# ViTAE-Transformer/LeMeViT

Hardware: AMD Instinct MI355X
Metric: images/sec LeMeViT-Base 224^2 bf16 fwd+bwd (higher is better)
Workload: dtype bf16; 1 GPU; lemevit_base 224x224 bf16-autocast train step (fwd+bwd+AdamW), batch 128/GPU, drop_path 0.1, random-init weights; global_batch=128, parallelism=dp1, launch=eager, weight-gradient GEMMs on a side stream

## Files before the change

### lemevit_amd/csrc/attn_mfma.hip

```cpp
#include <stdlib.h>
#include <atomic>
#include "common.h"
#include "attn_internal.h"

#ifndef LMV_XCD_REMAP
#define LMV_XCD_REMAP 1
#endif

namespace {

constexpr int D = 32;
typedef __attribute__((address_space(3))) bf16x4_t* lds4_t;

__device__ __forceinline__ int swz(int r, int c16) { return r * 64 + ((c16 ^ (((r >> 2) & 1) << 1)) << 4); }

template <int NTHREADS>
__device__ __forceinline__ void stage_rows2(unsigned char* sa, const bf16_t* ba, int64_t rsa, unsigned char* sb, const bf16_t* bb, int64_t rsb,
                                            int r0, int nrows, int L, int tid) {
  const int total = nrows * 4, last = max(L - 1, 0);
  for (int c0 = 0; c0 < total; c0 += NTHREADS * 4) {
    uint4 va[4], vb[4];
#pragma unroll
    for (int j = 0; j < 4; ++j) {
      const int c = min(c0 + j * NTHREADS + tid, total - 1), cc = c & 3;
      const int rr = min(r0 + (c >> 2), last);
      va[j] = *reinterpret_cast<const uint4*>(ba + (int64_t)rr * rsa + cc * 8);
      vb[j] = *reinterpret_cast<const uint4*>(bb + (int64_t)rr * rsb + cc * 8);
    }
#pragma unroll
    for (int j = 0; j < 4; ++j) {
      const int c = c0 + j * NTHREADS + tid, r = c >> 2, cc = c & 3;
      if (c >= total) continue;
      const bool ok = r0 + r < L;
      *reinterpret_cast<uint4*>(sa + swz(r, cc)) = ok ? va[j] : make_uint4(0, 0, 0, 0);
      *reinterpret_cast<uint4*>(sb + swz(r, cc)) = ok ? vb[j] : make_uint4(0, 0, 0, 0);
    }
  }
}

__device__ __forceinline__ bf16x8_t frag_n(const unsigned char* s, int row0, int lane) {
  return *reinterpret_cast<const bf16x8_t*>(s + swz(row0 + (lane & 15), lane >> 4));
}
__device__ __forceinline__ bf16x8_t frag_t(const unsigned char* s, int rowA, int rowB, int d0, int lane) {
  const int g = lane >> 4, i = lane & 15, rr = i >> 2, q = i & 3;
  const int ra = rowA + g * 4 + rr, rb = rowB + g * 4 + rr, c16 = q, off = (d0 >> 4) * 8;
  bf16x4_t lo = __builtin_amdgcn_ds_read_tr16_b64_v4bf16((lds4_t)(s + swz(ra, c16) + off));
  bf16x4_t hi = __builtin_amdgcn_ds_read_tr16_b64_v4bf16((lds4_t)(s + swz(rb, c16) + off));
  return __builtin_shufflevector(lo, hi, 0, 1, 2, 3, 4, 5, 6, 7);
}

__device__ __forceinline__ bf16x8_t pack8(const f32x4_t& a, const f32x4_t& b) {
  bf16x8_t r;
  r[0] = (__bf16)a[0]; r[1] = (__bf16)a[1]; r[2] = (__bf16)a[2]; r[3] = (__bf16)a[3];
  r[4] = (__bf16)b[0]; r[5] = (__bf16)b[1]; r[6] = (__bf16)b[2]; r[7] = (__bf16)b[3];
  return r;
}
__device__ __forceinline__ bf16x8_t load_frag_global(const bf16_t* base, int64_t rs, int row, int L, int lane) {
  uint4 v = make_uint4(0, 0, 0, 0);
  if (row < L) v = *reinterpret_cast<const uint4*>(base + (int64_t)row * rs + (lane >> 4) * 8);
  return __builtin_bit_cast(bf16x8_t, v);
}
__device__ __forceinline__ float group_max4(float v) { return lmv_xmax4(v); }
__device__ __forceinline__ float group_sum4(float v) { return lmv_xsum4(v); }
__device__ __forceinline__ void store4(bf16_t* p, const f32x4_t& v) { *reinterpret_cast<uint2*>(p) = make_uint2(pack_bf2(v[0], v[1]), pack_bf2(v[2], v[3])); }
__device__ __forceinline__ void store8(bf16_t* row, int g, const f32x4_t& x0, const f32x4_t& x1) {
  *reinterpret_cast<uint4*>(row + g * 8) = make_uint4(pack_bf2(x0[0], x0[1]), pack_bf2(x0[2], x0[3]), pack_bf2(x1[0], x1[1]), pack_bf2(x1[2], x1[3]));
}

#define MFMA(a, b, c) __builtin_amdgcn_mfma_f32_16x16x32_bf16(a, b, c, 0, 0, 0)

__device__ __forceinline__ int xcd_contiguous(int id, int n) {
  if (n & 7) return id;
  return (id & 7) * (n >> 3) + (id >> 3);
}

typedef __attribute__((ext_vector_type(8))) _Float16 f16x8_t;
typedef __attribute__((ext_vector_type(2))) _Float16 f16x2_t;

__device__ __forceinline__ unsigned bf2_to_h2(unsigned w) {
  const float lo = fminf(fmaxf(__uint_as_float(w << 16), -65504.f), 65504.f), hi = fminf(fmaxf(__uint_as_float(w & 0xffff0000u), -65504.f), 65504.f);
  return __builtin_bit_cast(unsigned, __builtin_amdgcn_cvt_pkrtz(lo, hi));
}
__device__ __forceinline__ f16x8_t pack8h(const f32x4_t& a, const f32x4_t& b) {
  typedef __attribute__((ext_vector_type(4))) unsigned u32x4_t;
  const u32x4_t w = {__builtin_bit_cast(unsigned, __builtin_amdgcn_cvt_pkrtz(a[0], a[1])), __builtin_bit_cast(unsigned, __builtin_amdgcn_cvt_pkrtz(a[2], a[3])),
                     __builtin_bit_cast(unsigned, __builtin_amdgcn_cvt_pkrtz(b[0], b[1])), __builtin_bit_cast(unsigned, __builtin_amdgcn_cvt_pkrtz(b[2], b[3]))};
  return __builtin_bit_cast(f16x8_t, w);
}

template <int NKT, int LK = 0, bool PV16 = false>
__device__ __forceinline__ void mfma_fwd_body(const AttnArgs& a, int qt_per_block, const int bx, const int h, const int b) {
  __shared__ __attribute__((aligned(16))) unsigned char sK[NKT * 16 * 64], sV[NKT * 16 * 64];
  const int tid = threadIdx.x, lane = tid & 63, wave = tid >> 6;
  const int Lk = LK ? LK : a.Lk;
  const bf16_t* qb = reinterpret_cast<const bf16_t*>(a.q) + b * a.q_bs + h * D;
  const bf16_t* kb = reinterpret_cast<const bf16_t*>(a.k) + b * a.k_bs + h * D;
  const bf16_t* vb = reinterpret_cast<const bf16_t*>(a.v) + b * a.v_bs + h * D;
  bf16_t* ob = reinterpret_cast<bf16_t*>(a.o) + b * a.o_bs + h * D;
  stage_rows2<256>(sK, kb, a.k_rs, sV, vb, a.v_rs, 0, NKT * 16, Lk, tid);
  __syncthreads();
  if constexpr (PV16) {
    for (int c = tid; c < NKT * 16 * 4; c += 256) {
      uint4 v = *reinterpret_cast<const uint4*>(sV + c * 16);
      v.x = bf2_to_h2(v.x); v.y = bf2_to_h2(v.y); v.z = bf2_to_h2(v.z); v.w = bf2_to_h2(v.w);
      *reinterpret_cast<uint4*>(sV + c * 16) = v;
    }
    __syncthreads();
  }
  const int nqt = (a.Lq + 15) >> 4;
  const int qt_end = min(nqt, (bx + 1) * qt_per_block);
  const int g = lane >> 4;
  const float sc2 = a.scale * 1.4426950408889634f;
  bf16x8_t qf_next = load_frag_global(qb, a.q_rs, (bx * qt_per_block + wave) * 16 + (lane & 15), a.Lq, lane);
  for (int qt = bx * qt_per_block + wave; qt < qt_end; qt += 4) {
    const int q = qt * 16 + (lane & 15);
    const bf16x8_t qf = qf_next;
    if (qt + 4 < qt_end) qf_next = load_frag_global(qb, a.q_rs, q + 64, a.Lq, lane);
    f32x4_t s[NKT];
    float m = -3e38f;
#pragma unroll
    for (int kt = 0; kt < NKT; ++kt) {
      if (LK && kt * 16 >= LK) { s[kt] = f32x4_t{-3e38f, -3e38f, -3e38f, -3e38f}; continue; }
      s[kt] = MFMA(frag_n(sK, kt * 16, lane), qf, (f32x4_t{0.f, 0.f, 0.f, 0.f}));
      if (kt * 16 + 16 > Lk) {
#pragma unroll
        for (int r = 0; r < 4; ++r)
          if (kt * 16 + g * 4 + r >= Lk) s[kt][r] = -3e38f;
      }
#pragma unroll
      for (int r = 0; r < 4; ++r) m = fmaxf(m, s[kt][r]);
    }
    m = group_max4(m);
    const float mc = m * sc2;
    float l = 0.f;
#pragma unroll
    for (int kt = 0; kt < NKT; ++kt) {
      if (LK && kt * 16 >= LK) { s[kt] = f32x4_t{0.f, 0.f, 0.f, 0.f}; continue; }
#pragma unroll
      for (int r = 0; r < 4; ++r) { const float p = __builtin_amdgcn_exp2f(fmaf(s[kt][r], sc2, -mc)); s[kt][r] = p; l += p; }
    }
    l = group_sum4(l);
    f32x4_t o0 = {0.f, 0.f, 0.f, 0.f}, o1 = {0.f, 0.f, 0.f, 0.f};
#pragma unroll
    for (int kb2 = 0; kb2 < NKT / 2; ++kb2) {
      if (LK && kb2 * 32 >= LK) continue;
      const bf16x8_t vt0 = frag_t(sV, kb2 * 32, kb2 * 32 + 16, 0, lane), vt1 = frag_t(sV, kb2 * 32, kb2 * 32 + 16, 16, lane);
      if constexpr (PV16) {
        const f16x8_t ph = pack8h(s[2 * kb2], s[2 * kb2 + 1]);
        o0 = __builtin_amdgcn_mfma_f32_16x16x32_f16(__builtin_bit_cast(f16x8_t, vt0), ph, o0, 0, 0, 0);
        o1 = __builtin_amdgcn_mfma_f32_16x16x32_f16(__builtin_bit_cast(f16x8_t, vt1), ph, o1, 0, 0, 0);
      } else {
        const bf16x8_t ph = pack8(s[2 * kb2], s[2 * kb2 + 1]);
        f32x4_t r0, r1;
#pragma unroll
        for (int r = 0; r < 4; ++r) { r0[r] = s[2 * kb2][r] - (float)ph[r]; r1[r] = s[2 * kb2 + 1][r] - (float)ph[4 + r]; }
        const bf16x8_t pl = pack8(r0, r1);
        o0 = MFMA(vt0, ph, o0); o0 = MFMA(vt0, pl, o0);
        o1 = MFMA(vt1, ph, o1); o1 = MFMA(vt1, pl, o1);
      }
    }
    if (q < a.Lq) {
      const float inv = 1.f / l;
      o0 *= inv; o1 *= inv;
      store8(ob + (int64_t)q * a.o_rs, g, o0, o1);
      if (a.lse && g == 0) a.lse[((int64_t)b * a.H + h) * a.Lq + q] = m * a.scale + __logf(l);
    }
  }
}

template <int NKT, int LK = 0, bool PV16 = false>
__global__ __launch_bounds__(256) void mfma_fwd_kernel(const AttnArgs a, int qt_per_block) {
  const int nb = gridDim.x, n = nb * a.H * a.B;
  const int L = LMV_XCD_REMAP ? xcd_contiguous((int)blockIdx.x + nb * ((int)blockIdx.y + a.H * (int)blockIdx.z), n) : (int)blockIdx.x + nb * ((int)blockIdx.y + a.H * (int)blockIdx.z);
  mfma_fwd_body<NKT, LK, PV16>(a, qt_per_block, L % nb, (L / nb) % a.H, L / (nb * a.H));
}

template <int NKT1, int LK1, int NKT2, int LK2>
__global__ __launch_bounds__(256) void mfma_fwd_pair_kernel(const AttnArgs a1, const AttnArgs a2, int per1, int per2, int nblk1) {
  const int n1 = nblk1 * a1.H * a1.B;
  int id = (int)blockIdx.x;
  if (id < n1 && LMV_XCD_REMAP) id = xcd_contiguous(id, n1);
  if (id < n1) { const int bx = id % nblk1, t = id / nblk1; mfma_fwd_body<NKT1, LK1, true>(a1, per1, bx, t % a1.H, t / a1.H); }
  else { const int t = id - n1; mfma_fwd_body<NKT2, LK2, true>(a2, per2, 0, t % a2.H, t / a2.H); }
}

template <int NKT>
__global__ __launch_bounds__(256) void mfma_bwd_dq_kernel(const AttnArgs a, float* __restrict__ delta, int qt_per_block) {
  __shared__ __attribute__((aligned(16))) unsigned char sK[NKT * 16 * 64], sV[NKT * 16 * 64];
  const int tid = threadIdx.x, lane = tid & 63, wave = tid >> 6, h = blockIdx.y, b = blockIdx.z;
  const bf16_t* qb = reinterpret_cast<const bf16_t*>(a.q) + b * a.q_bs + h * D;
  const bf16_t* gb = reinterpret_cast<const bf16_t*>(a.d_o) + b * a.o_bs + h * D;
  const bf16_t* ob = reinterpret_cast<const bf16_t*>(a.o) + b * a.o_bs + h * D;
  bf16_t* dqb = reinterpret_cast<bf16_t*>(a.dq) + b * a.q_bs + h * D;
  stage_rows2<256>(sK, reinterpret_cast<const bf16_t*>(a.k) + b * a.k_bs + h * D, a.k_rs, sV, reinterpret_cast<const bf16_t*>(a.v) + b * a.v_bs + h * D, a.v_rs, 0, NKT * 16, a.Lk, tid);
  __syncthreads();
  const int nqt = (a.Lq + 15) >> 4;
  const int qt_end = min(nqt, (int)(blockIdx.x + 1) * qt_per_block);
  const int g = lane >> 4;
  const int64_t bh = ((int64_t)b * a.H + h) * a.Lq;
  for (int qt = blockIdx.x * qt_per_block + wave; qt < qt_end; qt += 4) {
    const int q = qt * 16 + (lane & 15);
    const bool vq = q < a.Lq;
    const bf16x8_t qf = load_frag_global(qb, a.q_rs, q, a.Lq, lane);
    const bf16x8_t gf = load_frag_global(gb, a.o_rs, q, a.Lq, lane);
    const bf16x8_t of = load_frag_global(ob, a.o_rs, q, a.Lq, lane);
    const float lse = vq ? a.lse[bh + q] : 0.f;
    float dl = 0.f;
#pragma unroll
    for (int j = 0; j < 8; ++j) dl += (float)gf[j] * (float)of[j];
    dl = group_sum4(dl);
    if (vq && g == 0) delta[bh + q] = dl;
    f32x4_t dq0 = {0.f, 0.f, 0.f, 0.f}, dq1 = {0.f, 0.f, 0.f, 0.f};
#pragma unroll
    for (int kb2 = 0; kb2 < NKT / 2; ++kb2) {
      f32x4_t ds[2];
#pragma unroll
      for (int t = 0; t < 2; ++t) {
        const int kt = 2 * kb2 + t;
        const f32x4_t s = MFMA(frag_n(sK, kt * 16, lane), qf, (f32x4_t{0.f, 0.f, 0.f, 0.f}));
        const f32x4_t dp = MFMA(frag_n(sV, kt * 16, lane), gf, (f32x4_t{0.f, 0.f, 0.f, 0.f}));
#pragma unroll
        for (int r = 0; r < 4; ++r) {
          const bool ok = vq && (kt * 16 + g * 4 + r < a.Lk);
          const float p = ok ? __expf(s[r] * a.scale - lse) : 0.f;
          ds[t][r] = p * (dp[r] - dl) * a.scale;
        }
      }
      const bf16x8_t dsf = pack8(ds[0], ds[1]);
      dq0 = MFMA(frag_t(sK, kb2 * 32, kb2 * 32 + 16, 0, lane), dsf, dq0);
      dq1 = MFMA(frag_t(sK, kb2 * 32, kb2 * 32 + 16, 16, lane), dsf, dq1);
    }
    if (vq) {
      store8(dqb + (int64_t)q * a.q_rs, g, dq0, dq1);
    }
  }
}
// ... 364 lines not shown
    const float4 d0 = *reinterpret_cast<const float4*>(sDl + r0 + g * 4), d1 = *reinterpret_cast<const float4*>(sDl + r0 + 16 + g * 4);
    const float lse[8] = {l0.x, l0.y, l0.z, l0.w, l1.x, l1.y, l1.z, l1.w};
    const float dl[8] = {d0.x, d0.y, d0.z, d0.w, d1.x, d1.y, d1.z, d1.w};
#pragma unroll
    for (int i = 0; i < TPW; ++i) {
      const int kt = wave + i * 4;
      if (kt >= NKT || kt * 16 >= Lk) continue;
      const bool kvalid = kt * 16 + (lane & 15) < Lk;
      const f32x4_t s0 = MFMA(qn0, kf[i], (f32x4_t{0.f, 0.f, 0.f, 0.f})), s1 = MFMA(qn1, kf[i], (f32x4_t{0.f, 0.f, 0.f, 0.f}));
      const f32x4_t p0 = MFMA(gn0, vf[i], (f32x4_t{0.f, 0.f, 0.f, 0.f})), p1 = MFMA(gn1, vf[i], (f32x4_t{0.f, 0.f, 0.f, 0.f}));
      f32x4_t pr[2], ds[2];
#pragma unroll
      for (int r = 0; r < 4; ++r) {
        const float e0 = kvalid ? __expf(s0[r] * a.scale - lse[r]) : 0.f, e1 = kvalid ? __expf(s1[r] * a.scale - lse[4 + r]) : 0.f;
        pr[0][r] = e0; pr[1][r] = e1;
        ds[0][r] = e0 * (p0[r] - dl[r]) * a.scale; ds[1][r] = e1 * (p1[r] - dl[4 + r]) * a.scale;
      }
      const bf16x8_t pf = pack8(pr[0], pr[1]), dsf = pack8(ds[0], ds[1]);
      dv[i][0] = MFMA(gt0, pf, dv[i][0]); dv[i][1] = MFMA(gt1, pf, dv[i][1]);
      dk[i][0] = MFMA(qt0, dsf, dk[i][0]); dk[i][1] = MFMA(qt1, dsf, dk[i][1]);
      const uint4 w = __builtin_bit_cast(uint4, dsf);
      const int wsl = (g ^ ((lane >> 2) & 3)) * 8;
      *reinterpret_cast<uint2*>(sT(buf, wave, 0, i) + (lane & 15) * 32 + wsl) = make_uint2(w.x, w.y);
      *reinterpret_cast<uint2*>(sT(buf, wave, 1, i) + (lane & 15) * 32 + wsl) = make_uint2(w.z, w.w);
    }
    __syncthreads();
    {
      const int rr = (lane & 15) >> 2, qq = lane & 3;
      f32x4_t dq = {0.f, 0.f, 0.f, 0.f};
#pragma unroll
      for (int pp = 0; pp < NPAIR; ++pp) {
        const int kta = 2 * pp, ktb = 2 * pp + 1;
        if (kta * 16 >= Lk) continue;
        const bool has_b = ktb < NKT && ktb * 16 < Lk;
        const bf16x4_t lo = __builtin_amdgcn_ds_read_tr16_b64_v4bf16((lds4_t)(sT(buf, kta & 3, qt_w, kta >> 2) + (g * 4 + rr) * 32 + (qq ^ g) * 8));
        bf16x4_t hi = {(__bf16)0.f, (__bf16)0.f, (__bf16)0.f, (__bf16)0.f};
        if (has_b) hi = __builtin_amdgcn_ds_read_tr16_b64_v4bf16((lds4_t)(sT(buf, ktb & 3, qt_w, ktb >> 2) + (g * 4 + rr) * 32 + (qq ^ g) * 8));
        const bf16x8_t dst = __builtin_shufflevector(lo, hi, 0, 1, 2, 3, 4, 5, 6, 7);
        dq = MFMA(ktf[pp], dst, dq);
      }
      const int q = r0 + qt_w * 16 + (lane & 15);
      if (q < Lq) store4(dqb + (int64_t)q * a.q_rs + g * 8 + dh * 4, dq);
    }
  }
#pragma unroll
  for (int i = 0; i < TPW; ++i) {
    const int kt = wave + i * 4, key = kt * 16 + (lane & 15);
    if (kt >= NKT || key >= Lk) continue;
    store8(reinterpret_cast<bf16_t*>(a.dk) + b * a.k_bs + (int64_t)key * a.k_rs + h * D, g, dk[i][0], dk[i][1]);
    store8(reinterpret_cast<bf16_t*>(a.dv) + b * a.v_bs + (int64_t)key * a.v_rs + h * D, g, dv[i][0], dv[i][1]);
  }
}

template <int NKT, int LK = 0, int VER = 1>
__global__ __launch_bounds__(256, 2) void mfma_bwd_fused_kernel(const AttnArgs a) {
  const int n = a.H * a.B, id = (int)blockIdx.y + a.H * (int)blockIdx.z;
  const int L = LMV_XCD_REMAP ? xcd_contiguous(id, n) : id;
  if constexpr (VER == 2) mfma_bwd_fused_body2<NKT, LK>(a, L % a.H, L / a.H);
  else mfma_bwd_fused_body<NKT, LK>(a, L % a.H, L / a.H);
}

template <int NKT1, int LK1, int VER = 1>
__global__ __launch_bounds__(256, 2) void mfma_bwd_pair_kernel(const AttnArgs a1, const AttnArgs a2) {
  const int n1 = a1.H * a1.B;
  int id = (int)blockIdx.x;
  if (id < n1 && LMV_XCD_REMAP) id = xcd_contiguous(id, n1);
  if (id < n1) { if constexpr (VER == 2) mfma_bwd_fused_body2<NKT1, LK1>(a1, id % a1.H, id / a1.H); else mfma_bwd_fused_body<NKT1, LK1>(a1, id % a1.H, id / a1.H); }
  else mfma_bwd_dkv_body<2, 1, false, true, 16, 32>(a2, nullptr, nullptr, nullptr, 32, 0, (id - n1) % a2.H, (id - n1) / a2.H);
}

__global__ __launch_bounds__(256) void scatter_bf16_kernel(const float* __restrict__ acc, bf16_t* __restrict__ dst, int64_t bs, int64_t rs, int B, int H,
                                                          int L, int LP) {
  const unsigned idx = blockIdx.x * 256 + threadIdx.x, total = (unsigned)B * H * L * D;
  if (idx >= total) return;
  const unsigned d = idx % D, l = (idx / D) % L, h = (idx / (D * L)) % H, b = idx / (D * L * H);
  dst[b * bs + (int64_t)l * rs + h * D + d] = f2bf(acc[((((int64_t)b * H + h) * LP) + l) * D + d]);
}

__global__ __launch_bounds__(256) void scatter_sum_kernel(const float* __restrict__ acc0, const float* __restrict__ acc1, bf16_t* __restrict__ dst0,
                                                         bf16_t* __restrict__ dst1, int64_t bs0, int64_t rs0, int64_t bs1, int64_t rs1, int B, int H, int L,
                                                         int LP, int nslab) {
  const unsigned idx = blockIdx.x * 256 + threadIdx.x, per = (unsigned)B * H * L * (D / 4);
  if (idx >= 2 * per) return;
  const bool second = idx >= per;
  const unsigned i = second ? idx - per : idx;
  const unsigned d4 = i % (D / 4), l = (i / (D / 4)) % L, h = (i / ((D / 4) * L)) % H, b = i / ((D / 4) * L * H);
  const float* src = (second ? acc1 : acc0) + ((((int64_t)b * H + h) * LP) + l) * D + d4 * 4;
  const int64_t slab = (int64_t)B * H * LP * D;
  f32x4_t s = {0.f, 0.f, 0.f, 0.f};
  for (int k = 0; k < nslab; ++k) s += *reinterpret_cast<const f32x4_t*>(src + k * slab);
  bf16_t* dst = second ? dst1 + b * bs1 + (int64_t)l * rs1 + h * D + d4 * 4 : dst0 + b * bs0 + (int64_t)l * rs0 + h * D + d4 * 4;
  store4(dst, s);
}

constexpr int RKT = 8, RK = RKT * 16;
constexpr int RKT_B = 4, RKB = RKT_B * 16;

__global__ __launch_bounds__(256) void mfma_fwd_split_kernel(const AttnArgs a, float* __restrict__ part, int nsplit) {
  __shared__ __attribute__((aligned(16))) unsigned char sK[4 * RK * 64], sV[4 * RK * 64];
  const int tid = threadIdx.x, lane = tid & 63, wave = tid >> 6, g = lane >> 4;
  const int nbx = gridDim.x, Lid = LMV_XCD_REMAP ? xcd_contiguous((int)blockIdx.x + nbx * ((int)blockIdx.y + a.H * (int)blockIdx.z), nbx * a.H * a.B)
                                                 : (int)blockIdx.x + nbx * ((int)blockIdx.y + a.H * (int)blockIdx.z);
  const int bx = Lid % nbx, h = (Lid / nbx) % a.H, b = Lid / (nbx * a.H);
  const int split = bx * 4 + wave, k0 = split * RK;
  const bf16_t* kb = reinterpret_cast<const bf16_t*>(a.k) + b * a.k_bs + h * D;
  const bf16_t* vb = reinterpret_cast<const bf16_t*>(a.v) + b * a.v_bs + h * D;
  unsigned char* wK = sK + wave * RK * 64;
  unsigned char* wV = sV + wave * RK * 64;
  stage_rows2<64>(wK, kb, a.k_rs, wV, vb, a.v_rs, k0, RK, a.Lk, lane);
  asm volatile("s_waitcnt vmcnt(0) lgkmcnt(0)" ::: "memory");
  __builtin_amdgcn_wave_barrier();
  if (split >= nsplit) return;
  const int q = lane & 15;
  float* pp = part + ((((int64_t)b * a.H + h) * nsplit + split) * 16 + q) * (D + 2);
  if (k0 >= a.Lk) {
    if (g == 0) { pp[0] = -1e30f; pp[1] = 0.f; }
#pragma unroll
    for (int r = 0; r < 4; ++r) { pp[2 + g * 4 + r] = 0.f; pp[18 + g * 4 + r] = 0.f; }
    return;
  }
// ... 642 lines not shown
    else if (a.Lk == 49) hipLaunchKernelGGL((mfma_bwd_fused_kernel<4, 49>), grid, block, 0, st, a);
    else if (nkt == 4) hipLaunchKernelGGL((mfma_bwd_fused_kernel<4>), grid, block, 0, st, a);
    else if (nkt == 8) hipLaunchKernelGGL((mfma_bwd_fused_kernel<8>), grid, block, 0, st, a);
    else hipLaunchKernelGGL((mfma_bwd_fused_kernel<14>), grid, block, 0, st, a);
    LMV_CHECK_LAUNCH("attn_mfma_bwd_fused");
    return LMV_OK;
  }
  if (nkt == 14 && a.Lq > 16) {
    int nk, pr, lds;
    if (int rc = long_geometry(a, &nk, &pr, &lds)) return rc;
    hipLaunchKernelGGL(mfma_bwd_dq_long_kernel, dim3((nqt + pr - 1) / pr, a.H, a.B), dim3(256), lds, st, a, delta, pr, nk);
  } else if (nkt == 2 && fuse_dq) {
  } else {
    dim3 grid((nqt + per - 1) / per, a.H, a.B), block(256);
    switch (nkt) {
      case 2: hipLaunchKernelGGL((mfma_bwd_dq_kernel<2>), grid, block, 0, st, a, delta, per); break;
      case 4: hipLaunchKernelGGL((mfma_bwd_dq_kernel<4>), grid, block, 0, st, a, delta, per); break;
      case 8: hipLaunchKernelGGL((mfma_bwd_dq_kernel<8>), grid, block, 0, st, a, delta, per); break;
      default: hipLaunchKernelGGL((mfma_bwd_dq_kernel<14>), grid, block, 0, st, a, delta, per); break;
    }
  }
  int nsplit, qpb;
  dkv_split(a, &nsplit, &qpb);
  dim3 grid(nsplit, a.H, a.B), block(256);
  const size_t acc_elems = (size_t)nsplit * a.B * a.H * nkt * 16 * D;
  float* acc_k = acc; float* acc_v = acc + acc_elems;
  if (nsplit > 1) {
#define DKV(N, K) hipLaunchKernelGGL((mfma_bwd_dkv_kernel<N, K, true>), grid, block, 0, st, a, delta, acc_k, acc_v, qpb)
    if (nkt == 2 && fuse_dq && a.Lk == 16) hipLaunchKernelGGL((mfma_bwd_dkv_kernel<2, 1, true, true, 16>), grid, block, 0, st, a, delta, acc_k, acc_v, qpb);
    else if (nkt == 2 && fuse_dq) hipLaunchKernelGGL((mfma_bwd_dkv_kernel<2, 1, true, true>), grid, block, 0, st, a, delta, acc_k, acc_v, qpb);
    else
    switch (nkt) { case 2: DKV(2, 1); break; case 4: DKV(4, 2); break; case 8: DKV(8, 4); break; default: DKV(14, 4); break; }
#undef DKV
    const unsigned n = 2u * (unsigned)a.B * a.H * a.Lk * (D / 4);
    hipLaunchKernelGGL(scatter_sum_kernel, dim3((n + 255) / 256), dim3(256), 0, st, (const float*)acc_k, (const float*)acc_v, (bf16_t*)a.dk, (bf16_t*)a.dv,
                       a.k_bs, a.k_rs, a.v_bs, a.v_rs, a.B, a.H, a.Lk, nkt * 16, nsplit);
  } else {
#define DKV(N, K) hipLaunchKernelGGL((mfma_bwd_dkv_kernel<N, K, false>), grid, block, 0, st, a, delta, acc_k, acc_v, qpb)
    if (nkt == 2 && fuse_dq && a.Lk == 16) hipLaunchKernelGGL((mfma_bwd_dkv_kernel<2, 1, false, true, 16>), grid, block, 0, st, a, delta, acc_k, acc_v, qpb);
    else if (nkt == 2 && fuse_dq) hipLaunchKernelGGL((mfma_bwd_dkv_kernel<2, 1, false, true>), grid, block, 0, st, a, delta, acc_k, acc_v, qpb);
    else
    switch (nkt) { case 2: DKV(2, 1); break; case 4: DKV(4, 2); break; case 8: DKV(8, 4); break; default: DKV(14, 4); break; }
#undef DKV
  }
  LMV_CHECK_LAUNCH("attn_mfma_bwd");
  return LMV_OK;
}

int lmv_attn_mfma_fwd_pair(const AttnArgs& a1, const AttnArgs& a2, hipStream_t st) {
  const int on = lmv_config().attn_pair;
  if (!on || a1.B != a2.B || a1.H != a2.H || a2.Lk != 16 || a2.Lq != 16 || a1.Lq != a1.Lk || (a1.Lk != 196 && a1.Lk != 49)) return 0;
  const int per1 = qt_per_block_for(a1), nqt1 = (a1.Lq + 15) / 16, nblk1 = (nqt1 + per1 - 1) / per1;
  dim3 grid((nblk1 + 1) * a1.H * a1.B), block(256);
  if (a1.Lk == 196) hipLaunchKernelGGL((mfma_fwd_pair_kernel<14, 196, 2, 16>), grid, block, 0, st, a1, a2, per1, 1, nblk1);
  else hipLaunchKernelGGL((mfma_fwd_pair_kernel<4, 49, 2, 16>), grid, block, 0, st, a1, a2, per1, 1, nblk1);
  return 1;
}

int lmv_attn_mfma_bwd_pair(const AttnArgs& a1, const AttnArgs& a2, hipStream_t st) {
  const int on = lmv_config().attn_pair;
  if (!on || a1.B != a2.B || a1.H != a2.H || a2.Lk != 16 || a2.Lq != 16 || a1.Lq != a1.Lk || (a1.Lk != 196 && a1.Lk != 49)) return 0;
  dim3 grid(2 * a1.H * a1.B), block(256);
  const bool v2 = lmv_config().attn_fused_bwd == 2;
  if (a1.Lk == 196 && v2) hipLaunchKernelGGL((mfma_bwd_pair_kernel<14, 196, 2>), grid, block, 0, st, a1, a2);
  else if (v2) hipLaunchKernelGGL((mfma_bwd_pair_kernel<4, 49, 2>), grid, block, 0, st, a1, a2);
  else if (a1.Lk == 196) hipLaunchKernelGGL((mfma_bwd_pair_kernel<14, 196>), grid, block, 0, st, a1, a2);
  else hipLaunchKernelGGL((mfma_bwd_pair_kernel<4, 49>), grid, block, 0, st, a1, a2);
  return 1;
}
```

### lemevit_amd/csrc/common.h

```cpp
#pragma once
#include <hip/hip_runtime.h>
#include <stdint.h>
#include <stdio.h>
#include "../../include/lemevit_hip.h"

typedef unsigned short bf16_t;
typedef __attribute__((ext_vector_type(8))) __bf16 bf16x8_t;
typedef __attribute__((ext_vector_type(4))) __bf16 bf16x4_t;
typedef __attribute__((ext_vector_type(4))) float f32x4_t;

#define LMV_WAVE 64

void lmv_set_error(const char* fmt, ...);
#define LMV_FAIL(code, ...)          \
  do {                               \
    lmv_set_error(__VA_ARGS__);      \
    return (code);                   \
  } while (0)
unsigned* lmv_stage_errword(void* stream);
int lmv_stage_capacity(const void* kernel, int threads, size_t lds_bytes);

extern bool g_lmv_timing_on;
void lmv_timing_begin(void* stream, double flops, double bytes, int kind);
void lmv_timing_end(void* stream);
// ... 18 lines not shown
                                                                float* __restrict__ out_a, int na, float* __restrict__ out_b, int mode) {
  const int cx = threadIdx.x & 7, rg = threadIdx.x >> 3, i = (blk * 8 + cx) * 4;
  float4 a = make_float4(0.f, 0.f, 0.f, 0.f);
  if (i < width) {
    const float* p = partial + i;
    int r = rg;
    for (; r + 96 < nrows; r += 128) {
      const float4 v0 = *reinterpret_cast<const float4*>(p + (int64_t)r * width);
      const float4 v1 = *reinterpret_cast<const float4*>(p + (int64_t)(r + 32) * width);
      const float4 v2 = *reinterpret_cast<const float4*>(p + (int64_t)(r + 64) * width);
      const float4 v3 = *reinterpret_cast<const float4*>(p + (int64_t)(r + 96) * width);
      a.x += (v0.x + v1.x) + (v2.x + v3.x); a.y += (v0.y + v1.y) + (v2.y + v3.y);
      a.z += (v0.z + v1.z) + (v2.z + v3.z); a.w += (v0.w + v1.w) + (v2.w + v3.w);
    }
    for (; r < nrows; r += 32) {
      const float4 v = *reinterpret_cast<const float4*>(p + (int64_t)r * width);
      a.x += v.x; a.y += v.y; a.z += v.z; a.w += v.w;
    }
  }
  red[rg * 8 + cx] = a;
  __syncthreads();
  if (rg == 0 && i < width) {
#pragma unroll 8
    for (int k = 1; k < 32; ++k) { const float4 v = red[k * 8 + cx]; a.x += v.x; a.y += v.y; a.z += v.z; a.w += v.w; }
    const float s[4] = {a.x, a.y, a.z, a.w};
#pragma unroll
    for (int e = 0; e < 4; ++e) {
      const int j = i + e;
      if (mode == 0) { if (j < na) out_a[j] += s[e]; else out_b[j - na] += s[e]; }
      else { const int t = j / na, ch = j - t * na; if (t < 9) out_a[ch * 9 + t] += s[e]; else out_b[ch] += s[e]; }
    }
  }
}

struct LmvConfig {
  int gemm_bk;
  int gemm_bk32_tiles;
  int dw_bk;
  int dw_target_blocks;
  int gemm_no_dma;
  int gemm_w8;
  int gemm_cumap;
  int gemm_nst, gemm_nst_dw;
  int gemm_wn;
  int gemm_rs;
  int dwconv_v;
  int ln_exact_fused;
  int res_ln_fused;
  int dx_ln_fused;
  int mlp_split384;
  int mlp_rw96;
  int mlp_tm;
  int attn_pv16, attn_fuse_dq, attn_fused_bwd, attn_pair;
  int ln_bwd_blocks, ln_bwd_minrows;
  int stage_ticket_skew;
};
LmvConfig& lmv_config();

bool lmv_rs_eligible(const lmv_linear_problem* p, int nproblems, int N, int K, int act, bool force);
int lmv_rs_linear(const lmv_linear_problem* p, int nproblems, int N, int K, int act, hipStream_t st);
bool lmv_wn_eligible(const lmv_linear_problem* p, int nproblems, int N, int K, int act, bool force);
bool lmv_mlp_rw96_eligible(const lmv_mlp_problem* p, int nproblems, int C, int hidden);
int lmv_mlp_rw96_fwd(const lmv_mlp_problem* p, int nproblems, const lmv_mlp_weights* w, float eps, hipStream_t st);
int lmv_wn_linear(const lmv_linear_problem* p, int nproblems, int N, int K, int act, hipStream_t st);

static inline bool lmv_aligned16(const void* p) { return (((uintptr_t)p) & 15u) == 0; }

__device__ __forceinline__ float bf2f(bf16_t v) { return __uint_as_float(((unsigned)v) << 16); }
typedef __attribute__((ext_vector_type(2))) __bf16 bf16x2_t;
typedef __attribute__((ext_vector_type(2))) float f32x2_t;
__device__ __forceinline__ unsigned pack_bf2(float lo, float hi) {
  const f32x2_t f = {lo, hi};
  return __builtin_bit_cast(unsigned, __builtin_convertvector(f, bf16x2_t));
}
__device__ __forceinline__ bf16_t f2bf(float f) { return (bf16_t)(pack_bf2(f, 0.f) & 0xffffu); }

template <typename T> struct DT;
template <> struct DT<float> {
  static constexpr int EPC = 4;
  static __device__ __forceinline__ float ld(const float* p) { return *p; }
  static __device__ __forceinline__ void st(float* p, float v) { *p = v; }
};
template <> struct DT<bf16_t> {
  static constexpr int EPC = 8;
  static __device__ __forceinline__ float ld(const bf16_t* p) { return bf2f(*p); }
  static __device__ __forceinline__ void st(bf16_t* p, float v) { *p = f2bf(v); }
};

template <typename T> __device__ __forceinline__ void chunk_to_f(const uint4& c, float* f);
template <> __device__ __forceinline__ void chunk_to_f<float>(const uint4& c, float* f) {
  f[0] = __uint_as_float(c.x); f[1] = __uint_as_float(c.y); f[2] = __uint_as_float(c.z); f[3] = __uint_as_float(c.w);
}
template <> __device__ __forceinline__ void chunk_to_f<bf16_t>(const uint4& c, float* f) {
  f[0] = __uint_as_float(c.x << 16); f[1] = __uint_as_float(c.x & 0xffff0000u);
  f[2] = __uint_as_float(c.y << 16); f[3] = __uint_as_float(c.y & 0xffff0000u);
  f[4] = __uint_as_float(c.z << 16); f[5] = __uint_as_float(c.z & 0xffff0000u);
  f[6] = __uint_as_float(c.w << 16); f[7] = __uint_as_float(c.w & 0xffff0000u);
}
template <typename T> __device__ __forceinline__ uint4 f_to_chunk(const float* f);
template <> __device__ __forceinline__ uint4 f_to_chunk<float>(const float* f) {
  return make_uint4(__float_as_uint(f[0]), __float_as_uint(f[1]), __float_as_uint(f[2]), __float_as_uint(f[3]));
}
template <> __device__ __forceinline__ uint4 f_to_chunk<bf16_t>(const float* f) {
  return make_uint4(pack_bf2(f[0], f[1]), pack_bf2(f[2], f[3]), pack_bf2(f[4], f[5]), pack_bf2(f[6], f[7]));
}

// ... 68 lines not shown
```

### lemevit_amd/csrc/misc.hip

```cpp
#include <stdarg.h>
#include <string.h>
#include <mutex>
#include <vector>
#include "common.h"

static thread_local char g_err[512] = "";

void lmv_set_error(const char* fmt, ...) {
  va_list ap;
  va_start(ap, fmt);
  vsnprintf(g_err, sizeof(g_err), fmt, ap);
  va_end(ap);
}
extern "C" const char* lmv_last_error(void) { return g_err; }

namespace {
struct ErrWord { unsigned* host = nullptr; unsigned* dev = nullptr; };
ErrWord g_errword[64];
std::mutex g_errword_mu;
}
unsigned* lmv_stage_errword(void* stream) {
  int dev = 0;
  (void)hipGetDevice(&dev);
  std::lock_guard<std::mutex> lock(g_errword_mu);
// ... 42 lines not shown
size_t g_timing_n = 0;
}
void lmv_timing_begin(void* stream, double flops, double bytes, int kind) {
  if (g_timing_n >= g_timing.size()) return;
  TimingRec& r = g_timing[g_timing_n];
  r.flops = flops; r.bytes = bytes; r.kind = kind;
  (void)hipEventRecord(r.e0, (hipStream_t)stream);
}
void lmv_timing_end(void* stream) {
  if (g_timing_n >= g_timing.size()) return;
  (void)hipEventRecord(g_timing[g_timing_n++].e1, (hipStream_t)stream);
}
void lmv_timing_set_kind(int kind) {
  if (g_timing_n < g_timing.size()) g_timing[g_timing_n].kind = kind;
}
extern "C" int lmv_debug_launch_timing(int capacity) {
  g_lmv_timing_on = false;
  for (auto& r : g_timing) { (void)hipEventDestroy(r.e0); (void)hipEventDestroy(r.e1); }
  g_timing.clear(); g_timing_n = 0;
  if (capacity <= 0) return LMV_OK;
  g_timing.resize((size_t)capacity);
  for (auto& r : g_timing)
    if (hipEventCreate(&r.e0) != hipSuccess || hipEventCreate(&r.e1) != hipSuccess) LMV_FAIL(LMV_ERR_LAUNCH, "launch timing: cannot create events");
  g_lmv_timing_on = true;
  return LMV_OK;
}
extern "C" int lmv_debug_launch_timing_read(float* ms, double* flops, double* bytes, int* kinds, int capacity) {
  g_lmv_timing_on = false;
  int n = 0;
  for (size_t i = 0; i < g_timing_n && n < capacity; ++i) {
    float t = 0.f;
    if (hipEventElapsedTime(&t, g_timing[i].e0, g_timing[i].e1) != hipSuccess) continue;
    ms[n] = t; flops[n] = g_timing[i].flops; bytes[n] = g_timing[i].bytes; kinds[n] = g_timing[i].kind; ++n;
  }
  return n;
}

extern "C" int lmv_abi_version(void) { return LMV_ABI_VERSION; }

#include <stdlib.h>
#include <string.h>
namespace {
int env_int(const char* name, int dflt) { const char* e = name ? getenv(name) : nullptr; return e && *e ? atoi(e) : dflt; }
struct ConfigKey { const char* key; const char* env; int LmvConfig::*field; int dflt; };
const ConfigKey kConfigKeys[] = {
    {"gemm_bk", nullptr, &LmvConfig::gemm_bk, 0}, {"gemm_bk32_tiles", nullptr, &LmvConfig::gemm_bk32_tiles, 512},
    {"dw_bk", nullptr, &LmvConfig::dw_bk, 32}, {"dw_target_blocks", "LMV_DW_TARGET_BLOCKS", &LmvConfig::dw_target_blocks, 0},
    {"gemm_no_dma", nullptr, &LmvConfig::gemm_no_dma, 0}, {"gemm_w8", "LMV_GEMM_W8", &LmvConfig::gemm_w8, 1},
    {"gemm_cumap", nullptr, &LmvConfig::gemm_cumap, 1}, {"gemm_nst", nullptr, &LmvConfig::gemm_nst, 2},
    {"gemm_nst_dw", nullptr, &LmvConfig::gemm_nst_dw, 3}, {"gemm_rs", "LMV_GEMM_RS", &LmvConfig::gemm_rs, 1}, {"gemm_wn", "LMV_GEMM_WN", &LmvConfig::gemm_wn, 1},
    {"dwconv_v", nullptr, &LmvConfig::dwconv_v, 0},
    {"stage_ticket_skew", "LMV_STAGE_TICKET_SKEW", &LmvConfig::stage_ticket_skew, 0}, {"mlp_tm", nullptr, &LmvConfig::mlp_tm, 0}, {"mlp_rw96", nullptr, &LmvConfig::mlp_rw96, 1}, {"mlp_split384", nullptr, &LmvConfig::mlp_split384, 1}, {"dx_ln_fused", nullptr, &LmvConfig::dx_ln_fused, 1}, {"res_ln_fused", nullptr, &LmvConfig::res_ln_fused, 1}, {"ln_exact_fused", nullptr, &LmvConfig::ln_exact_fused, 1}, {"attn_pv16", nullptr, &LmvConfig::attn_pv16, 1},
    {"attn_fuse_dq", nullptr, &LmvConfig::attn_fuse_dq, 1}, {"attn_fused_bwd", nullptr, &LmvConfig::attn_fused_bwd, 2},
    {"attn_pair", nullptr, &LmvConfig::attn_pair, 1}, {"ln_bwd_blocks", nullptr, &LmvConfig::ln_bwd_blocks, 1024},
    {"ln_bwd_minrows", nullptr, &LmvConfig::ln_bwd_minrows, 2},
};
LmvConfig config_from_env() {
  LmvConfig c{};
  for (const ConfigKey& k : kConfigKeys) c.*(k.field) = env_int(k.env, k.dflt);
  if (c.ln_bwd_blocks <= 0 || c.ln_bwd_blocks > 2048) c.ln_bwd_blocks = 512;
  if (c.ln_bwd_minrows <= 0) c.ln_bwd_minrows = 2;
  return c;
}
LmvConfig g_config = config_from_env();
}
LmvConfig& lmv_config() { return g_config; }
extern "C" int lmv_config_set(const char* key, int value) {
  if (!key) LMV_FAIL(LMV_ERR_SHAPE, "config_set: null key");
  for (const ConfigKey& k : kConfigKeys)
    if (!strcmp(k.key, key)) { g_config.*(k.field) = value; return LMV_OK; }
  LMV_FAIL(LMV_ERR_SHAPE, "config_set: unknown key '%s'", key);
}
extern "C" int lmv_config_get(const char* key, int* value) {
  if (!key || !value) LMV_FAIL(LMV_ERR_SHAPE, "config_get: null argument");
  for (const ConfigKey& k : kConfigKeys)
    if (!strcmp(k.key, key)) { *value = g_config.*(k.field); return LMV_OK; }
  LMV_FAIL(LMV_ERR_SHAPE, "config_get: unknown key '%s'", key);
}

namespace {

constexpr int TPB = 256;
inline int grid_for(int64_t work_items) {
  int64_t b = (work_items + TPB - 1) / TPB;
  if (b > 2048) b = 2048;
  if (b < 1) b = 1;
  return (int)b;
}

template <typename S, typename D>
__global__ __launch_bounds__(TPB) void cast_kernel(const S* __restrict__ src, D* __restrict__ dst, int64_t n) {
  const int64_t n4 = n >> 2;
  for (int64_t i = blockIdx.x * (int64_t)TPB + threadIdx.x; i < n4; i += (int64_t)gridDim.x * TPB) {
    float f[4];
    ld4(src + i * 4, f);
    st4(dst + i * 4, f);
  }
  if (blockIdx.x == 0 && threadIdx.x < (n & 3)) {
    const int64_t i = (n4 << 2) + threadIdx.x;
    DT<D>::st(dst + i, DT<S>::ld(src + i));
  }
}

struct RowScaleSeg { const void* x; const float* scale; void* y; unsigned chunks, cpr, rps; };
struct RowScaleArgs { RowScaleSeg s[2]; unsigned total; };

template <typename T>
// ... 441 lines not shown
```

Before: 4349 images/sec.

## Add fused attention backward v3 and in-stage V fp16 conversion for paired kernels

Introduces a new fused backward body (VER 3) for the paired attention kernel. It keeps K/V fragments in registers, stages Q, dO and K^T in LDS, and computes dQ through double-buffered transposed dS tiles shared across waves, alongside the dK/dV accumulation. The forward pair kernel now converts V to fp16 while staging it, which removes a separate LDS pass and its extra barrier. Both paths are enabled by default through a new attn_pair_v config (default 2), at the cost of more LDS use and a more complex kernel that may lower occupancy.

```diff
diff --git a/lemevit_amd/csrc/attn_mfma.hip b/lemevit_amd/csrc/attn_mfma.hip
--- a/lemevit_amd/csrc/attn_mfma.hip
+++ b/lemevit_amd/csrc/attn_mfma.hip
@@ -14,7 +14,8 @@
 
 __device__ __forceinline__ int swz(int r, int c16) { return r * 64 + ((c16 ^ (((r >> 2) & 1) << 1)) << 4); }
 
-template <int NTHREADS>
+__device__ __forceinline__ unsigned bf2_to_h2(unsigned w);
+template <int NTHREADS, bool CVTB = false>
 __device__ __forceinline__ void stage_rows2(unsigned char* sa, const bf16_t* ba, int64_t rsa, unsigned char* sb, const bf16_t* bb, int64_t rsb,
                                             int r0, int nrows, int L, int tid) {
   const int total = nrows * 4, last = max(L - 1, 0);
@@ -32,6 +33,7 @@
       const int c = c0 + j * NTHREADS + tid, r = c >> 2, cc = c & 3;
       if (c >= total) continue;
       const bool ok = r0 + r < L;
+      if constexpr (CVTB) { vb[j].x = bf2_to_h2(vb[j].x); vb[j].y = bf2_to_h2(vb[j].y); vb[j].z = bf2_to_h2(vb[j].z); vb[j].w = bf2_to_h2(vb[j].w); }
       *reinterpret_cast<uint4*>(sa + swz(r, cc)) = ok ? va[j] : make_uint4(0, 0, 0, 0);
       *reinterpret_cast<uint4*>(sb + swz(r, cc)) = ok ? vb[j] : make_uint4(0, 0, 0, 0);
     }
@@ -88,7 +90,7 @@
   return __builtin_bit_cast(f16x8_t, w);
 }
 
-template <int NKT, int LK = 0, bool PV16 = false>
+template <int NKT, int LK = 0, bool PV16 = false, bool VIN = false>
 __device__ __forceinline__ void mfma_fwd_body(const AttnArgs& a, int qt_per_block, const int bx, const int h, const int b) {
   __shared__ __attribute__((aligned(16))) unsigned char sK[NKT * 16 * 64], sV[NKT * 16 * 64];
   const int tid = threadIdx.x, lane = tid & 63, wave = tid >> 6;
@@ -97,9 +99,9 @@
   const bf16_t* kb = reinterpret_cast<const bf16_t*>(a.k) + b * a.k_bs + h * D;
   const bf16_t* vb = reinterpret_cast<const bf16_t*>(a.v) + b * a.v_bs + h * D;
   bf16_t* ob = reinterpret_cast<bf16_t*>(a.o) + b * a.o_bs + h * D;
-  stage_rows2<256>(sK, kb, a.k_rs, sV, vb, a.v_rs, 0, NKT * 16, Lk, tid);
+  stage_rows2<256, PV16 && VIN>(sK, kb, a.k_rs, sV, vb, a.v_rs, 0, NKT * 16, Lk, tid);
   __syncthreads();
-  if constexpr (PV16) {
+  if constexpr (PV16 && !VIN) {
     for (int c = tid; c < NKT * 16 * 4; c += 256) {
       uint4 v = *reinterpret_cast<const uint4*>(sV + c * 16);
       v.x = bf2_to_h2(v.x); v.y = bf2_to_h2(v.y); v.z = bf2_to_h2(v.z); v.w = bf2_to_h2(v.w);
@@ -175,13 +177,13 @@
   mfma_fwd_body<NKT, LK, PV16>(a, qt_per_block, L % nb, (L / nb) % a.H, L / (nb * a.H));
 }
 
-template <int NKT1, int LK1, int NKT2, int LK2>
+template <int NKT1, int LK1, int NKT2, int LK2, bool VIN = false>
 __global__ __launch_bounds__(256) void mfma_fwd_pair_kernel(const AttnArgs a1, const AttnArgs a2, int per1, int per2, int nblk1) {
   const int n1 = nblk1 * a1.H * a1.B;
   int id = (int)blockIdx.x;
   if (id < n1 && LMV_XCD_REMAP) id = xcd_contiguous(id, n1);
-  if (id < n1) { const int bx = id % nblk1, t = id / nblk1; mfma_fwd_body<NKT1, LK1, true>(a1, per1, bx, t % a1.H, t / a1.H); }
-  else { const int t = id - n1; mfma_fwd_body<NKT2, LK2, true>(a2, per2, 0, t % a2.H, t / a2.H); }
+  if (id < n1) { const int bx = id % nblk1, t = id / nblk1; mfma_fwd_body<NKT1, LK1, true, VIN>(a1, per1, bx, t % a1.H, t / a1.H); }
+  else { const int t = id - n1; mfma_fwd_body<NKT2, LK2, true, VIN>(a2, per2, 0, t % a2.H, t / a2.H); }
 }
 
 template <int NKT>
@@ -652,6 +654,140 @@
   }
 }
 
+template <int NKT, int LK>
+__device__ __forceinline__ void mfma_bwd_fused_body3(const AttnArgs& a, const int h, const int b) {
+  constexpr int TPW = (NKT + 3) / 4;
+  constexpr int NPAIR = (NKT + 1) / 2;
+  constexpr int NQ = NKT * 16;
+  constexpr int NCH = (NQ * 4 + 255) / 256;
+  constexpr int TBUF = 4 * 2 * TPW * 512;
+  static_assert(NQ % 32 == 0 && NQ <= 256, "one LSE row per thread, whole 32-query blocks");
+  __shared__ __attribute__((aligned(16))) unsigned char sQ[NQ * 64], sG[NQ * 64];
+  __shared__ __attribute__((aligned(16))) unsigned char sKT[(2 * TBUF > NQ * 64) ? 2 * TBUF : NQ * 64];
+  __shared__ __attribute__((aligned(16))) float sL[NQ], sDl[NQ];
+  auto sT = [&](int buf, int w, int t, int slot) -> unsigned char* { return &sKT[buf * TBUF + ((w * 2 + t) * TPW + slot) * 512]; };
+  const int tid = threadIdx.x, lane = tid & 63, wave = __builtin_amdgcn_readfirstlane(tid >> 6);
+  const int g = lane >> 4;
+  constexpr int Lk = LK;
+  const int Lq = a.Lq;
+  const int64_t bh = ((int64_t)b * a.H + h) * Lq;
+  const float sc2 = a.scale * 1.4426950408889634f;
+  const bf16_t* qb = reinterpret_cast<const bf16_t*>(a.q) + b * a.q_bs + h * D;
+  const bf16_t* kb = reinterpret_cast<const bf16_t*>(a.k) + b * a.k_bs + h * D;
+  const bf16_t* vb = reinterpret_cast<const bf16_t*>(a.v) + b * a.v_bs + h * D;
+  const bf16_t* gb = reinterpret_cast<const bf16_t*>(a.d_o) + b * a.o_bs + h * D;
+  const bf16_t* ob = reinterpret_cast<const bf16_t*>(a.o) + b * a.o_bs + h * D;
+  uint4 cq[NCH], cg[NCH], co[NCH], ck[NCH];
+#pragma unroll
+  for (int j = 0; j < NCH; ++j) {
+    const int c = min(j * 256 + tid, NQ * 4 - 1), cc = c & 3;
+    const int rq = min(c >> 2, Lq - 1), rk = min(c >> 2, Lk - 1);
+    cq[j] = *reinterpret_cast<const uint4*>(qb + (int64_t)rq * a.q_rs + cc * 8);
+    cg[j] = *reinterpret_cast<const uint4*>(gb + (int64_t)rq * a.o_rs + cc * 8);
+    co[j] = *reinterpret_cast<const uint4*>(ob + (int64_t)rq * a.o_rs + cc * 8);
+    ck[j] = *reinterpret_cast<const uint4*>(kb + (int64_t)rk * a.k_rs + cc * 8);
+  }
+  const float lse_raw = a.lse[bh + min(tid, Lq - 1)];
+  bf16x8_t kf[TPW], vf[TPW];
+  f32x4_t dk[TPW][2], dv[TPW][2];
+#pragma unroll
+  for (int i = 0; i < TPW; ++i) {
+    const int kt = wave + i * 4;
+    kf[i] = load_frag_global(kb, a.k_rs, kt * 16 + (lane & 15), (kt < NKT) ? Lk : 0, lane);
+    vf[i] = load_frag_global(vb, a.v_rs, kt * 16 + (lane & 15), (kt < NKT) ? Lk : 0, lane);
+#pragma unroll
+    for (int dt = 0; dt < 2; ++dt) { dk[i][dt] = f32x4_t{0.f, 0.f, 0.f, 0.f}; dv[i][dt] = f32x4_t{0.f, 0.f, 0.f, 0.f}; }
+  }
+  if (tid < NQ) sL[tid] = tid < Lq ? lse_raw * 1.4426950408889634f : 1e30f;
+#pragma unroll
+  for (int j = 0; j < NCH; ++j) {
+    const int c = j * 256 + tid, r = c >> 2, cc = c & 3;
+    float gv[8], ov[8], dl = 0.f;
+    chunk_to_f<bf16_t>(cg[j], gv); chunk_to_f<bf16_t>(co[j], ov);
+#pragma unroll
+    for (int e = 0; e < 8; ++e) dl = fmaf(gv[e], ov[e], dl);
+    dl += __shfl_xor(dl, 1, 64);
+    dl += __shfl_xor(dl, 2, 64);
+    if ((NQ * 4) % 256 == 0 || c < NQ * 4) {
+      const bool okq = r < Lq, okk = r < Lk;
+      *reinterpret_cast<uint4*>(sQ + swz(r, cc)) = okq ? cq[j] : make_uint4(0, 0, 0, 0);
+      *reinterpret_cast<uint4*>(sG + swz(r, cc)) = okq ? cg[j] : make_uint4(0, 0, 0, 0);
+      *reinterpret_cast<uint4*>(sKT + swz(r, cc)) = okk ? ck[j] : make_uint4(0, 0, 0, 0);
+      if (cc == 0) sDl[r] = okq ? dl * a.scale : 0.f;
+    }
+  }
+  __syncthreads();
+  const int qt_w = wave >> 1, dh = wave & 1;
+  bf16x8_t ktf[NPAIR];
+#pragma unroll
+  for (int pp = 0; pp < NPAIR; ++pp) {
+    const int rowb = (2 * pp + 1 < NKT) ? (2 * pp + 1) * 16 : 2 * pp * 16;
+    ktf[pp] = frag_t(sKT, 2 * pp * 16, rowb, dh * 16, lane);
+  }
+  __syncthreads();
+  bf16_t* dqb = reinterpret_cast<bf16_t*>(a.dq) + b * a.q_bs + h * D;
+  int buf = 0;
+  for (int r0 = 0; r0 < NQ; r0 += 32, buf ^= 1) {
+    if (r0 >= Lq) break;
+    const bf16x8_t qn0 = frag_n(sQ, r0, lane), qn1 = frag_n(sQ, r0 + 16, lane);
+    const bf16x8_t gn0 = frag_n(sG, r0, lane), gn1 = frag_n(sG, r0 + 16, lane);
+    const bf16x8_t qt0 = frag_t(sQ, r0, r0 + 16, 0, lane), qt1 = frag_t(sQ, r0, r0 + 16, 16, lane);
+    const bf16x8_t gt0 = frag_t(sG, r0, r0 + 16, 0, lane), gt1 = frag_t(sG, r0, r0 + 16, 16, lane);
+    const float4 l0 = *reinterpret_cast<const float4*>(sL + r0 + g * 4), l1 = *reinterpret_cast<const float4*>(sL + r0 + 16 + g * 4);
+    const float4 d0 = *reinterpret_cast<const float4*>(sDl + r0 + g * 4), d1 = *reinterpret_cast<const float4*>(sDl + r0 + 16 + g * 4);
+    const float lse[8] = {l0.x, l0.y, l0.z, l0.w, l1.x, l1.y, l1.z, l1.w};
+    const float dl[8] = {d0.x, d0.y, d0.z, d0.w, d1.x, d1.y, d1.z, d1.w};
+#pragma unroll
+    for (int i = 0; i < TPW; ++i) {
+      const int kt = wave + i * 4;
+      if (kt >= NKT || kt * 16 >= Lk) continue;
+      const bool kvalid = kt * 16 + (lane & 15) < Lk;
+      const f32x4_t s0 = MFMA(qn0, kf[i], (f32x4_t{0.f, 0.f, 0.f, 0.f})), s1 = MFMA(qn1, kf[i], (f32x4_t{0.f, 0.f, 0.f, 0.f}));
+      const f32x4_t p0 = MFMA(gn0, vf[i], (f32x4_t{0.f, 0.f, 0.f, 0.f})), p1 = MFMA(gn1, vf[i], (f32x4_t{0.f, 0.f, 0.f, 0.f}));
+      f32x4_t pr[2], ds[2];
+#pragma unroll
+      for (int r = 0; r < 4; ++r) {
+        const float e0 = kvalid ? __builtin_amdgcn_exp2f(fmaf(s0[r], sc2, -lse[r])) : 0.f;
+        const float e1 = kvalid ? __builtin_amdgcn_exp2f(fmaf(s1[r], sc2, -lse[4 + r])) : 0.f;
+        pr[0][r] = e0; pr[1][r] = e1;
+        ds[0][r] = e0 * fmaf(p0[r], a.scale, -dl[r]); ds[1][r] = e1 * fmaf(p1[r], a.scale, -dl[4 + r]);
+      }
+      const bf16x8_t pf = pack8(pr[0], pr[1]), dsf = pack8(ds[0], ds[1]);
+      dv[i][0] = MFMA(gt0, pf, dv[i][0]); dv[i][1] = MFMA(gt1, pf, dv[i][1]);
+      dk[i][0] = MFMA(qt0, dsf, dk[i][0]); dk[i][1] = MFMA(qt1, dsf, dk[i][1]);
+      const uint4 w = __builtin_bit_cast(uint4, dsf);
+      const int wsl = (g ^ ((lane >> 2) & 3)) * 8;
+      *reinterpret_cast<uint2*>(sT(buf, wave, 0, i) + (lane & 15) * 32 + wsl) = make_uint2(w.x, w.y);
+      *reinterpret_cast<uint2*>(sT(buf, wave, 1, i) + (lane & 15) * 32 + wsl) = make_uint2(w.z, w.w);
+    }
+    __syncthreads();
+    {
+      const int rr = (lane & 15) >> 2, qq = lane & 3;
+      f32x4_t dq = {0.f, 0.f, 0.f, 0.f};
+#pragma unroll
+      for (int pp = 0; pp < NPAIR; ++pp) {
+        const int kta = 2 * pp, ktb = 2 * pp + 1;
+        if (kta * 16 >= Lk) continue;
+        const bool has_b = ktb < NKT && ktb * 16 < Lk;
+        const bf16x4_t lo = __builtin_amdgcn_ds_read_tr16_b64_v4bf16((lds4_t)(sT(buf, kta & 3, qt_w, kta >> 2) + (g * 4 + rr) * 32 + (qq ^ g) * 8));
+        bf16x4_t hi = {(__bf16)0.f, (__bf16)0.f, (__bf16)0.f, (__bf16)0.f};
+        if (has_b) hi = __builtin_amdgcn_ds_read_tr16_b64_v4bf16((lds4_t)(sT(buf, ktb & 3, qt_w, ktb >> 2) + (g * 4 + rr) * 32 + (qq ^ g) * 8));
+        const bf16x8_t dst = __builtin_shufflevector(lo, hi, 0, 1, 2, 3, 4, 5, 6, 7);
+        dq = MFMA(ktf[pp], dst, dq);
+      }
+      const int q = r0 + qt_w * 16 + (lane & 15);
+      if (q < Lq) store4(dqb + (int64_t)q * a.q_rs + g * 8 + dh * 4, dq);
+    }
+  }
+#pragma unroll
+  for (int i = 0; i < TPW; ++i) {
+    const int kt = wave + i * 4, key = kt * 16 + (lane & 15);
+    if (kt >= NKT || key >= Lk) continue;
+    store8(reinterpret_cast<bf16_t*>(a.dk) + b * a.k_bs + (int64_t)key * a.k_rs + h * D, g, dk[i][0], dk[i][1]);
+    store8(reinterpret_cast<bf16_t*>(a.dv) + b * a.v_bs + (int64_t)key * a.v_rs + h * D, g, dv[i][0], dv[i][1]);
+  }
+}
+
 template <int NKT, int LK = 0, int VER = 1>
 __global__ __launch_bounds__(256, 2) void mfma_bwd_fused_kernel(const AttnArgs a) {
   const int n = a.H * a.B, id = (int)blockIdx.y + a.H * (int)blockIdx.z;
@@ -665,7 +801,11 @@
   const int n1 = a1.H * a1.B;
   int id = (int)blockIdx.x;
   if (id < n1 && LMV_XCD_REMAP) id = xcd_contiguous(id, n1);
-  if (id < n1) { if constexpr (VER == 2) mfma_bwd_fused_body2<NKT1, LK1>(a1, id % a1.H, id / a1.H); else mfma_bwd_fused_body<NKT1, LK1>(a1, id % a1.H, id / a1.H); }
+  if (id < n1) {
+    if constexpr (VER == 3) mfma_bwd_fused_body3<NKT1, LK1>(a1, id % a1.H, id / a1.H);
+    else if constexpr (VER == 2) mfma_bwd_fused_body2<NKT1, LK1>(a1, id % a1.H, id / a1.H);
+    else mfma_bwd_fused_body<NKT1, LK1>(a1, id % a1.H, id / a1.H);
+  }
   else mfma_bwd_dkv_body<2, 1, false, true, 16, 32>(a2, nullptr, nullptr, nullptr, 32, 0, (id - n1) % a2.H, (id - n1) / a2.H);
 }
 
@@ -1414,7 +1554,10 @@
   if (!on || a1.B != a2.B || a1.H != a2.H || a2.Lk != 16 || a2.Lq != 16 || a1.Lq != a1.Lk || (a1.Lk != 196 && a1.Lk != 49)) return 0;
   const int per1 = qt_per_block_for(a1), nqt1 = (a1.Lq + 15) / 16, nblk1 = (nqt1 + per1 - 1) / per1;
   dim3 grid((nblk1 + 1) * a1.H * a1.B), block(256);
-  if (a1.Lk == 196) hipLaunchKernelGGL((mfma_fwd_pair_kernel<14, 196, 2, 16>), grid, block, 0, st, a1, a2, per1, 1, nblk1);
+  const bool vin = lmv_config().attn_pair_v >= 2;
+  if (a1.Lk == 196 && vin) hipLaunchKernelGGL((mfma_fwd_pair_kernel<14, 196, 2, 16, true>), grid, block, 0, st, a1, a2, per1, 1, nblk1);
+  else if (vin) hipLaunchKernelGGL((mfma_fwd_pair_kernel<4, 49, 2, 16, true>), grid, block, 0, st, a1, a2, per1, 1, nblk1);
+  else if (a1.Lk == 196) hipLaunchKernelGGL((mfma_fwd_pair_kernel<14, 196, 2, 16>), grid, block, 0, st, a1, a2, per1, 1, nblk1);
   else hipLaunchKernelGGL((mfma_fwd_pair_kernel<4, 49, 2, 16>), grid, block, 0, st, a1, a2, per1, 1, nblk1);
   return 1;
 }
@@ -1423,8 +1566,10 @@
   const int on = lmv_config().attn_pair;
   if (!on || a1.B != a2.B || a1.H != a2.H || a2.Lk != 16 || a2.Lq != 16 || a1.Lq != a1.Lk || (a1.Lk != 196 && a1.Lk != 49)) return 0;
   dim3 grid(2 * a1.H * a1.B), block(256);
-  const bool v2 = lmv_config().attn_fused_bwd == 2;
-  if (a1.Lk == 196 && v2) hipLaunchKernelGGL((mfma_bwd_pair_kernel<14, 196, 2>), grid, block, 0, st, a1, a2);
+  const bool v2 = lmv_config().attn_fused_bwd == 2, v3 = v2 && lmv_config().attn_pair_v >= 2;
+  if (a1.Lk == 196 && v3) hipLaunchKernelGGL((mfma_bwd_pair_kernel<14, 196, 3>), grid, block, 0, st, a1, a2);
+  else if (v3) hipLaunchKernelGGL((mfma_bwd_pair_kernel<4, 49, 3>), grid, block, 0, st, a1, a2);
+  else if (a1.Lk == 196 && v2) hipLaunchKernelGGL((mfma_bwd_pair_kernel<14, 196, 2>), grid, block, 0, st, a1, a2);
   else if (v2) hipLaunchKernelGGL((mfma_bwd_pair_kernel<4, 49, 2>), grid, block, 0, st, a1, a2);
   else if (a1.Lk == 196) hipLaunchKernelGGL((mfma_bwd_pair_kernel<14, 196>), grid, block, 0, st, a1, a2);
   else hipLaunchKernelGGL((mfma_bwd_pair_kernel<4, 49>), grid, block, 0, st, a1, a2);
diff --git a/lemevit_amd/csrc/common.h b/lemevit_amd/csrc/common.h
--- a/lemevit_amd/csrc/common.h
+++ b/lemevit_amd/csrc/common.h
@@ -94,6 +94,7 @@
   int mlp_rw96;
   int mlp_tm;
   int attn_pv16, attn_fuse_dq, attn_fused_bwd, attn_pair;
+  int attn_pair_v;
   int ln_bwd_blocks, ln_bwd_minrows;
   int stage_ticket_skew;
 };
diff --git a/lemevit_amd/csrc/misc.hip b/lemevit_amd/csrc/misc.hip
--- a/lemevit_amd/csrc/misc.hip
+++ b/lemevit_amd/csrc/misc.hip
@@ -118,7 +118,7 @@
     {"dwconv_v", nullptr, &LmvConfig::dwconv_v, 0},
     {"stage_ticket_skew", "LMV_STAGE_TICKET_SKEW", &LmvConfig::stage_ticket_skew, 0}, {"mlp_tm", nullptr, &LmvConfig::mlp_tm, 0}, {"mlp_rw96", nullptr, &LmvConfig::mlp_rw96, 1}, {"mlp_split384", nullptr, &LmvConfig::mlp_split384, 1}, {"dx_ln_fused", nullptr, &LmvConfig::dx_ln_fused, 1}, {"res_ln_fused", nullptr, &LmvConfig::res_ln_fused, 1}, {"ln_exact_fused", nullptr, &LmvConfig::ln_exact_fused, 1}, {"attn_pv16", nullptr, &LmvConfig::attn_pv16, 1},
     {"attn_fuse_dq", nullptr, &LmvConfig::attn_fuse_dq, 1}, {"attn_fused_bwd", nullptr, &LmvConfig::attn_fused_bwd, 2},
-    {"attn_pair", nullptr, &LmvConfig::attn_pair, 1}, {"ln_bwd_blocks", nullptr, &LmvConfig::ln_bwd_blocks, 1024},
+    {"attn_pair", nullptr, &LmvConfig::attn_pair, 1}, {"attn_pair_v", "LMV_ATTN_PAIR_V", &LmvConfig::attn_pair_v, 2}, {"ln_bwd_blocks", nullptr, &LmvConfig::ln_bwd_blocks, 1024},
     {"ln_bwd_minrows", nullptr, &LmvConfig::ln_bwd_minrows, 2},
 };
 LmvConfig config_from_env() {
```

Result: no change. 4363 images/sec, median of 6 (+0.3%).
